# flupkede/codesearch

Hardware: AMD Instinct MI355X
Metric: chunks embedded+searched/sec over 10M×384 corpus; recall@10 vs CPU ref (higher is better)
Workload: dtype f32

## Files before the change

codesearch_amd/csrc/attention_shx_body.hpp:

```cpp
#pragma once

#include "encoder.hpp"
#include "split_f16.hpp"

#ifndef AT_STAMP
#define AT_STAMP(i)
#endif
#ifndef CS_ATTN_ARITH
#define CS_ATTN_ARITH 2
#endif
#ifndef CS_ATTN_LAZY_RESCALE
#define CS_ATTN_LAZY_RESCALE 4.0f
#endif
#ifndef CS_ATTN_PIPE_FENCE
#define CS_ATTN_PIPE_FENCE __builtin_amdgcn_sched_barrier(0)
#endif

namespace cs {

typedef __fp16 h16x2 __attribute__((ext_vector_type(2)));

constexpr float kLog2e = 1.4426950408889634f;
constexpr float kMaskedLog2 = -3.0e38f;

union Frag8 {
    f16x8 v;
    uint32_t u[4];
    uint2 d[2];
};

typedef short s16x4 __attribute__((ext_vector_type(4)));

union FragTr {
    f16x8 v;
    s16x4 q[2];
};

__device__ __forceinline__ void split_pair_rtz_ng(float a, float b, uint32_t& hi, uint32_t& lo) {
    const h16x2 h = __builtin_amdgcn_cvt_pkrtz(a, b);
    const h16x2 l = __builtin_amdgcn_cvt_pkrtz((a - (float)h[0]) * kShLoScale, (b - (float)h[1]) * kShLoScale);
    hi = __builtin_bit_cast(uint32_t, h);
    lo = __builtin_bit_cast(uint32_t, l);
}

__device__ __forceinline__ float mix_residual_lo(float e, uint32_t hpair) {
    float r;
    asm("v_fma_mix_f32 %0, %1, -1.0, %2 op_sel_hi:[1,0,0]" : "=v"(r) : "v"(hpair), "v"(e));
    return r;
}
__device__ __forceinline__ float mix_residual_hi(float e, uint32_t hpair) {
    float r;
    asm("v_fma_mix_f32 %0, %1, -1.0, %2 op_sel:[1,0,0] op_sel_hi:[1,0,0]" : "=v"(r) : "v"(hpair), "v"(e));
    return r;
}

__device__ __forceinline__ float xhalf_max_swap(float t) {
    const uint32_t u = __builtin_bit_cast(uint32_t, t);
    const auto r = __builtin_amdgcn_permlane32_swap(u, u, false, false);
    const uint32_t a = r[0], b = r[1];
    return fmaxf(__builtin_bit_cast(float, a), __builtin_bit_cast(float, b));
}

struct AttnMemPlain {
    __device__ __forceinline__ f16x8 ld16(const _Float16* p) const { return *reinterpret_cast<const f16x8*>(p); }
    __device__ __forceinline__ f16x8 stage_load(const _Float16* src, char* lds_piece) const { sh_glds16(src, lds_piece); return f16x8{}; }
    __device__ __forceinline__ void stage_store(char*, int, f16x8) const {}
    __device__ __forceinline__ void st8(_Float16* p, f16x4 v) const { *reinterpret_cast<f16x4*>(p) = v; }
};

template <int NC, class MQ, class MO, int POS = 0, int PIPE = 0>
__device__ __forceinline__ void
attention_shx_body(char* smem, const MQ& mq, const MO& mo, const _Float16* qkvs, const int32_t* __restrict__ mask,
                   _Float16* ctxs, uint32_t* __restrict__ flag, uint32_t L, uint32_t H,
                   float scale_log2e, uint32_t HB, float* __restrict__ range_out,
                   const uint32_t* __restrict__ seq_unit, const uint32_t* __restrict__ unit_len,
                   uint32_t bx, uint32_t by, uint32_t bz, uint32_t gx, uint32_t gz, const float* __restrict__ alibi_log2 = nullptr,
                   uint32_t window = 0) {
    constexpr bool ALIBI = POS == 1, WINDOW = POS == 2;
    constexpr bool IMM = PIPE >= 2;
    constexpr bool EARLY = PIPE == 3;
    const float wlimit = (float)window;
    constexpr int KT = 128;
    const uint32_t Lp = (L + 31) & ~31u;
    char* Kt = smem;
    char* Vt = Kt + (size_t)NC * KT * 128;
    float* madd = reinterpret_cast<float*>(Vt + (size_t)NC * KT * 128);
    int* last_valid_p = reinterpret_cast<int*>(madd + Lp);
    const int tid = threadIdx.x, lane = tid & 63;
    const int wave = __builtin_amdgcn_readfirstlane(tid >> 6);
    const int l31 = lane & 31, h = lane >> 5;
    const uint32_t wq = 4 / HB, hsub = (uint32_t)wave / wq, qt = (uint32_t)wave % wq;
    const uint32_t head = bx * HB + hsub, b = by, qb = bz;
    Kt += (size_t)hsub * (KT / HB) * 128;
    Vt += (size_t)hsub * (KT / HB) * 128;
    const uint32_t nh = H / (32 * NC), nch = 3 * nh * NC;
    const _Float16* base = qkvs + (size_t)b * L * nch * 64;
    bool ovf = false;

    AT_STAMP(0);
    if (tid == 0) *last_valid_p = 0;

    const int kswz = (l31 >> 1) & 7;
    int k_hi[2], k_lo[2];
#pragma unroll
    for (int s = 0; s < 2; ++s) {
        k_hi[s] = ((2 * s + h) ^ kswz) * 16;
        k_lo[s] = ((4 + 2 * s + h) ^ kswz) * 16;
    }
    const int vq = (lane & 15) >> 2, vp = lane & 3, vg = (lane >> 4) & 1;
    const int vfv = 4 * ((vq >> 1) & 1);
    const int v_hi = (4 * h + vq) * 128 + (((2 * vg + (vp >> 1)) ^ vfv) * 16) + 8 * (vp & 1);
    const int v_lo = v_hi ^ 64;

    const bool wave_live = qb * 128 + qt * 32 < L;
    const uint32_t query = qb * 128 + qt * 32 + l31;
    const uint32_t qsrc = query < L ? query : L - 1;
    float neg_slope = 0.0f;
    const float qpos = (float)query - (float)(4 * h);
    if constexpr (ALIBI) neg_slope = -alibi_log2[head];
    f16x8 qh[NC][2], ql[NC][2];
#pragma unroll
    for (int c = 0; c < NC; ++c) {
        const _Float16* qp = base + ((size_t)qsrc * nch + head * NC + c) * 64 + 8 * h;
#pragma unroll
        for (int s = 0; s < 2; ++s) {
            qh[c][s] = mq.ld16(qp + 16 * s);
            ql[c][s] = mq.ld16(qp + 32 + 16 * s);
        }
    }
#if CS_ATTN_ARITH == 2 && !defined(CS_ATTN_SCALAR_SOFTMAX)
    f16x8 qhs[NC][2];
#pragma unroll
    for (int c = 0; c < NC; ++c)
#pragma unroll
        for (int s = 0; s < 2; ++s) {
            qhs[c][s] = qh[c][s] * (_Float16)kShLoInv;
            ql[c][s] = ql[c][s] * (_Float16)kShLoInv;
        }
#endif
    sh_f32x16 ohh[NC], oxx[NC];
#pragma unroll
    for (int c = 0; c < NC; ++c)
#pragma unroll
        for (int r = 0; r < 16; ++r) { ohh[c][r] = 0.0f; oxx[c][r] = 0.0f; }
    float m = -__builtin_huge_valf(), lsum = 0.0f;

    auto stage = [&](uint32_t st) {
        const uint32_t live = Lp - st * KT < (uint32_t)KT ? Lp - st * KT : (uint32_t)KT;
        for (uint32_t i0 = qt; i0 < live / 8; i0 += 4 * wq) {
            f16x8 rk[4][NC], rv[4][NC];
#pragma unroll
            for (int u = 0; u < 4; ++u) {
                const uint32_t ii = i0 + u * wq;
                if (ii < live / 8) {
                    const uint32_t row = ii * 8 + (lane >> 3);
                    const uint32_t gk = st * KT + row;
                    const uint32_t key = gk < L ? gk : L - 1;
                    const uint32_t ck = (lane & 7) ^ ((row >> 1) & 7);
                    const uint32_t cv = (lane & 7) ^ (4 * ((row >> 1) & 1));
#pragma unroll
                    for (int c = 0; c < NC; ++c) {
                        rk[u][c] = mq.stage_load(base + ((size_t)key * nch + (nh + head) * NC + c) * 64 + ck * 8, Kt + (size_t)c * KT * 128 + ii * 1024);
                        rv[u][c] = mq.stage_load(base + ((size_t)key * nch + (2 * nh + head) * NC + c) * 64 + cv * 8, Vt + (size_t)c * KT * 128 + ii * 1024);
                    }
                }
            }
#pragma unroll
            for (int u = 0; u < 4; ++u) {
                const uint32_t ii = i0 + u * wq;
                if (ii < live / 8) {
#pragma unroll
                    for (int c = 0; c < NC; ++c) {
                        mq.stage_store(Kt + (size_t)c * KT * 128 + ii * 1024, lane, rk[u][c]);
                        mq.stage_store(Vt + (size_t)c * KT * 128 + ii * 1024, lane, rv[u][c]);
                    }
                }
            }
        }
    };
    stage(0);
    __syncthreads();
    for (uint32_t key = tid; key < Lp; key += 256) {
        const bool ok = key < L && mask[(size_t)b * L + key] != 0;
        madd[key] = ok ? 0.0f : kMaskedLog2;
        if (ok) atomicMax(last_valid_p, (int)key);
    }
    asm volatile("s_waitcnt vmcnt(0)" ::: "memory");
    __syncthreads();
    const uint32_t ntiles = (uint32_t)(*last_valid_p) / 32 + 1;

    typedef __attribute__((address_space(3))) char* lds_char_p;
    typedef __attribute__((address_space(3))) const f16x8* lds_f16x8_cp;
    typedef __attribute__((address_space(3))) const sh_f32x4* lds_f32x4_cp;
    uint32_t ka[4] = {0, 0, 0, 0}, va[2] = {0, 0}, ma0 = 0;
    if constexpr (IMM) {
        const uint32_t k0 = (uint32_t)(uintptr_t)(lds_char_p)Kt + (uint32_t)l31 * 128u, v0 = (uint32_t)(uintptr_t)(lds_char_p)Vt;
#pragma unroll
        for (int s = 0; s < 2; ++s) { ka[s] = k0 + (uint32_t)k_hi[s]; ka[2 + s] = k0 + (uint32_t)k_lo[s]; }
        va[0] = v0 + (uint32_t)v_hi;
        va[1] = v0 + (uint32_t)v_lo;
        ma0 = (uint32_t)(uintptr_t)(lds_char_p)reinterpret_cast<char*>(madd) + 16u * (uint32_t)h;
#pragma unroll
        for (int i = 0; i < 4; ++i) asm volatile("" : "+v"(ka[i]));
        asm volatile("" : "+v"(va[0]), "+v"(va[1]), "+v"(ma0));
    }

    for (uint32_t st = 0; st * 4 < ntiles; ++st) {
        if constexpr (WINDOW) {
            if (st * KT > qb * 128 + 127 + window || st * KT + (KT - 1) + window < qb * 128) continue;
        }
        if (st > 0) {
            __syncthreads();
            stage(st);
            asm volatile("s_waitcnt vmcnt(0)" ::: "memory");
            __syncthreads();
        }
        if (!wave_live) continue;
        const uint32_t kt_end = ntiles - st * 4 < 4 ? ntiles - st * 4 : 4;
        const uint32_t ma_st = ma0 + st * 512u;
        uint32_t kl_lo = 0, kl_hi = kt_end;
        if constexpr (WINDOW) {
            const int q0 = (int)(qb * 128 + qt * 32), w = (int)window, t0 = (int)(st * 4);
            const int first = q0 - 31 - w > 0 ? (q0 - 31 - w + 31) / 32 : 0, past = (q0 + 31 + w) / 32 + 1;
            kl_lo = (uint32_t)(first > t0 ? first - t0 : 0);
            kl_hi = past - t0 < (int)kt_end ? (uint32_t)(past - t0 > 0 ? past - t0 : 0) : kt_end;
        }
        auto compute_s = [&](uint32_t kl, sh_f32x16& hh, sh_f32x16& xx) __attribute__((always_inline)) {
#pragma unroll
            for (int r = 0; r < 16; ++r) { hh[r] = 0.0f; xx[r] = 0.0f; }
            if constexpr (EARLY) {
                f16x8 kf[NC][4];
#pragma unroll
                for (int c = 0; c < NC; ++c)
#pragma unroll
                    for (int i = 0; i < 4; ++i) kf[c][i] = *(lds_f16x8_cp)(uintptr_t)(ka[i] + (uint32_t)(c * KT * 128) + kl * 4096u);
                __builtin_amdgcn_sched_barrier(0);
#pragma unroll
                for (int c = 0; c < NC; ++c)
#pragma unroll
                    for (int s = 0; s < 2; ++s) {
                        hh = __builtin_amdgcn_mfma_f32_32x32x16_f16(kf[c][s], qh[c][s], hh, 0, 0, 0);
#if CS_ATTN_ARITH == 2 && !defined(CS_ATTN_SCALAR_SOFTMAX)
                        hh = __builtin_amdgcn_mfma_f32_32x32x16_f16(kf[c][s], ql[c][s], hh, 0, 0, 0);
                        hh = __builtin_amdgcn_mfma_f32_32x32x16_f16(kf[c][2 + s], qhs[c][s], hh, 0, 0, 0);
#else
                        xx = __builtin_amdgcn_mfma_f32_32x32x16_f16(kf[c][s], ql[c][s], xx, 0, 0, 0);
                        xx = __builtin_amdgcn_mfma_f32_32x32x16_f16(kf[c][2 + s], qh[c][s], xx, 0, 0, 0);
#endif
                    }
                return;
            }
#pragma unroll
            for (int c = 0; c < NC; ++c) {
                const char* kr = Kt + (size_t)c * KT * 128 + (size_t)(kl * 32 + l31) * 128;
#pragma unroll
                for (int s = 0; s < 2; ++s) {
                    f16x8 kh, kl8;
                    if constexpr (IMM) {
                        kh = *(lds_f16x8_cp)(uintptr_t)(ka[s] + (uint32_t)(c * KT * 128) + kl * 4096u);
                        kl8 = *(lds_f16x8_cp)(uintptr_t)(ka[2 + s] + (uint32_t)(c * KT * 128) + kl * 4096u);
                    } else {
                        kh = *reinterpret_cast<const f16x8*>(kr + k_hi[s]);
                        kl8 = *reinterpret_cast<const f16x8*>(kr + k_lo[s]);
                    }
                    hh = __builtin_amdgcn_mfma_f32_32x32x16_f16(kh, qh[c][s], hh, 0, 0, 0);
#if CS_ATTN_ARITH == 2 && !defined(CS_ATTN_SCALAR_SOFTMAX)
                    hh = __builtin_amdgcn_mfma_f32_32x32x16_f16(kh, ql[c][s], hh, 0, 0, 0);
                    hh = __builtin_amdgcn_mfma_f32_32x32x16_f16(kl8, qhs[c][s], hh, 0, 0, 0);
#else
                    xx = __builtin_amdgcn_mfma_f32_32x32x16_f16(kh, ql[c][s], xx, 0, 0, 0);
                    xx = __builtin_amdgcn_mfma_f32_32x32x16_f16(kl8, qh[c][s], xx, 0, 0, 0);
#endif
                }
            }
        };
        auto finish_tile = [&](uint32_t kl, sh_f32x16& hh, sh_f32x16& xx) __attribute__((always_inline)) {
            const uint32_t kt = st * 4 + kl;
#ifndef CS_ATTN_SCALAR_SOFTMAX
            sh_f32x2 p2[8];
            float tmax = -__builtin_huge_valf();
            const sh_f32x2 lo_inv2 = {kShLoInv, kShLoInv}, scale2 = {scale_log2e, scale_log2e};
#pragma unroll
            for (int g = 0; g < 4; ++g) {
                sh_f32x4 ma;
                if constexpr (IMM) ma = *(lds_f32x4_cp)(uintptr_t)(ma_st + (kl * 32u + 8u * g) * 4u);
                else ma = *reinterpret_cast<const sh_f32x4*>(madd + kt * 32 + 8 * g + 4 * h);
#pragma unroll
                for (int e2 = 0; e2 < 2; ++e2) {
                    const int r = 4 * g + 2 * e2;
                    const sh_f32x2 x2 = {xx[r], xx[r + 1]}, h2 = {hh[r], hh[r + 1]};
                    sh_f32x2 m2 = {ma[2 * e2], ma[2 * e2 + 1]};
                    if constexpr (ALIBI) {
                        const float d0 = qpos - (float)(kt * 32 + 8 * g + 2 * e2);
                        m2[0] = fmaf(neg_slope, fabsf(d0), m2[0]);
                        m2[1] = fmaf(neg_slope, fabsf(d0 - 1.0f), m2[1]);
                    }
                    if constexpr (WINDOW) {
                        const float d0 = qpos - (float)(kt * 32 + 8 * g + 2 * e2);
                        m2[0] = fabsf(d0) > wlimit ? kMaskedLog2 : m2[0];
                        m2[1] = fabsf(d0 - 1.0f) > wlimit ? kMaskedLog2 : m2[1];
                    }
#if CS_ATTN_ARITH == 2
                    (void)x2; (void)lo_inv2;
                    const sh_f32x2 s2 = __builtin_elementwise_fma(h2, scale2, m2);
#else
                    const sh_f32x2 s2 = __builtin_elementwise_fma(__builtin_elementwise_fma(x2, lo_inv2, h2), scale2, m2);
#endif
                    p2[r / 2] = s2;
                    tmax = fmaxf(tmax, fmaxf(s2[0], s2[1]));
                }
            }
            if constexpr (IMM) tmax = xhalf_max_swap(tmax);
            else tmax = fmaxf(tmax, __shfl_xor(tmax, 32, 64));
#if CS_ATTN_ARITH == 2
            if (__any(tmax > m + CS_ATTN_LAZY_RESCALE)) {
#else
            if (__any(tmax > m)) {
#endif
                const float mnew = fmaxf(m, tmax);
                const float alpha = __builtin_amdgcn_exp2f(m - mnew);
                lsum *= alpha;
#pragma unroll
                for (int c = 0; c < NC; ++c)
#pragma unroll
                    for (int r = 0; r < 16; ++r) { ohh[c][r] *= alpha; oxx[c][r] *= alpha; }
                m = mnew;
            }
            typedef __attribute__((address_space(3))) s16x4* lds_s16x4_p;
            FragTr vhe[NC][2], vle[NC][2];
            if constexpr (EARLY) {
#pragma unroll
                for (int c = 0; c < NC; ++c)
#pragma unroll
                    for (int s = 0; s < 2; ++s) {
                        const uint32_t off = (uint32_t)(c * KT * 128) + kl * 4096u + (uint32_t)(s * 16 * 128);
                        vhe[c][s].q[0] = __builtin_amdgcn_ds_read_tr16_b64_v4i16((lds_s16x4_p)(uintptr_t)(va[0] + off));
                        vhe[c][s].q[1] = __builtin_amdgcn_ds_read_tr16_b64_v4i16((lds_s16x4_p)(uintptr_t)(va[0] + off + 1024u));
                        vle[c][s].q[0] = __builtin_amdgcn_ds_read_tr16_b64_v4i16((lds_s16x4_p)(uintptr_t)(va[1] + off));
                        vle[c][s].q[1] = __builtin_amdgcn_ds_read_tr16_b64_v4i16((lds_s16x4_p)(uintptr_t)(va[1] + off + 1024u));
                    }
                __builtin_amdgcn_sched_barrier(0);
            }
#if CS_ATTN_ARITH == 2
            const sh_f32x2 m2v = {m - 11.0f, m - 11.0f};
#else
            const sh_f32x2 m2v = {m, m};
#endif
            sh_f32x2 ps2 = {0.0f, 0.0f};
            Frag8 ph[2], pl[2];
            const sh_f32x2 lo_scale2 = {kShLoScale, kShLoScale};
#pragma unroll
            for (int i = 0; i < 8; ++i) {
                const sh_f32x2 d2 = p2[i] - m2v;
                const sh_f32x2 e2 = {__builtin_amdgcn_exp2f(d2[0]), __builtin_amdgcn_exp2f(d2[1])};
                ps2 += e2;
                const h16x2 hi = __builtin_amdgcn_cvt_pkrtz(e2[0], e2[1]);
#if CS_ATTN_ARITH == 2
                (void)lo_scale2;
                const uint32_t hib = __builtin_bit_cast(uint32_t, hi);
                const h16x2 lo = __builtin_amdgcn_cvt_pkrtz(mix_residual_lo(e2[0], hib), mix_residual_hi(e2[1], hib));
#else
                const sh_f32x2 back = {(float)hi[0], (float)hi[1]};
                const sh_f32x2 r2 = (e2 - back) * lo_scale2;
                const h16x2 lo = __builtin_amdgcn_cvt_pkrtz(r2[0], r2[1]);
#endif
                ph[i >> 2].u[i & 3] = __builtin_bit_cast(uint32_t, hi);
                pl[i >> 2].u[i & 3] = __builtin_bit_cast(uint32_t, lo);
            }
            lsum += ps2[0] + ps2[1];
#else
            float tmax = -__builtin_huge_valf();
#pragma unroll
            for (int g = 0; g < 4; ++g) {
                const sh_f32x4 ma = *reinterpret_cast<const sh_f32x4*>(madd + kt * 32 + 8 * g + 4 * h);
#pragma unroll
                for (int e = 0; e < 4; ++e) {
                    const int r = 4 * g + e;
                    float me = ma[e];
                    if constexpr (ALIBI) me = fmaf(neg_slope, fabsf(qpos - (float)(kt * 32 + 8 * g + e)), me);
                    if constexpr (WINDOW) me = fabsf(qpos - (float)(kt * 32 + 8 * g + e)) > wlimit ? kMaskedLog2 : me;
                    hh[r] = fmaf(fmaf(xx[r], kShLoInv, hh[r]), scale_log2e, me);
                    tmax = fmaxf(tmax, hh[r]);
                }
            }
            tmax = fmaxf(tmax, __shfl_xor(tmax, 32, 64));
            if (__any(tmax > m)) {
                const float mnew = fmaxf(m, tmax);
                const float alpha = __builtin_amdgcn_exp2f(m - mnew);
                lsum *= alpha;
#pragma unroll
                for (int c = 0; c < NC; ++c)
#pragma unroll
                    for (int r = 0; r < 16; ++r) { ohh[c][r] *= alpha; oxx[c][r] *= alpha; }
                m = mnew;
            }
            float psum = 0.0f;
#pragma unroll
            for (int r = 0; r < 16; ++r) {
                hh[r] = __builtin_amdgcn_exp2f(hh[r] - m);
                psum += hh[r];
            }
            lsum += psum;
            Frag8 ph[2], pl[2];
#pragma unroll
            for (int s = 0; s < 2; ++s)
#pragma unroll
                for (int w2 = 0; w2 < 4; ++w2) {
#ifdef CS_ATTN_P_HI_ONLY
                    const f16x2 pr = __builtin_convertvector(sh_f32x2{hh[8 * s + 2 * w2], hh[8 * s + 2 * w2 + 1]}, f16x2);
                    ph[s].u[w2] = __builtin_bit_cast(uint32_t, pr);
                    pl[s].u[w2] = 0u;
#else
                    split_pair_rtz_ng(hh[8 * s + 2 * w2], hh[8 * s + 2 * w2 + 1], ph[s].u[w2], pl[s].u[w2]);
#endif
                }
#endif
#ifdef CS_ATTN_SCALAR_SOFTMAX
            typedef __attribute__((address_space(3))) s16x4* lds_s16x4_p;
            FragTr vhe[NC][2], vle[NC][2];
#endif
#pragma unroll
            for (int c = 0; c < NC; ++c) {
                const char* vr = Vt + (size_t)c * KT * 128 + (size_t)kl * 32 * 128;
#pragma unroll
                for (int s = 0; s < 2; ++s) {
                    FragTr vh, vl;
                    if constexpr (EARLY) {
                        vh = vhe[c][s];
                        vl = vle[c][s];
                    } else if constexpr (IMM) {
                        const uint32_t off = (uint32_t)(c * KT * 128) + kl * 4096u + (uint32_t)(s * 16 * 128);
                        vh.q[0] = __builtin_amdgcn_ds_read_tr16_b64_v4i16((lds_s16x4_p)(uintptr_t)(va[0] + off));
                        vh.q[1] = __builtin_amdgcn_ds_read_tr16_b64_v4i16((lds_s16x4_p)(uintptr_t)(va[0] + off + 1024u));
                        vl.q[0] = __builtin_amdgcn_ds_read_tr16_b64_v4i16((lds_s16x4_p)(uintptr_t)(va[1] + off));
                        vl.q[1] = __builtin_amdgcn_ds_read_tr16_b64_v4i16((lds_s16x4_p)(uintptr_t)(va[1] + off + 1024u));
                    } else {
                    vh.q[0] = __builtin_amdgcn_ds_read_tr16_b64_v4i16((lds_s16x4_p)(vr + s * 16 * 128 + v_hi));
                    vh.q[1] = __builtin_amdgcn_ds_read_tr16_b64_v4i16((lds_s16x4_p)(vr + s * 16 * 128 + 8 * 128 + v_hi));
                    vl.q[0] = __builtin_amdgcn_ds_read_tr16_b64_v4i16((lds_s16x4_p)(vr + s * 16 * 128 + v_lo));
                    vl.q[1] = __builtin_amdgcn_ds_read_tr16_b64_v4i16((lds_s16x4_p)(vr + s * 16 * 128 + 8 * 128 + v_lo));
                    }
                    ohh[c] = __builtin_amdgcn_mfma_f32_32x32x16_f16(vh.v, ph[s].v, ohh[c], 0, 0, 0);
#if CS_ATTN_ARITH == 2 && !defined(CS_ATTN_SCALAR_SOFTMAX)
                    ohh[c] = __builtin_amdgcn_mfma_f32_32x32x16_f16(vh.v, pl[s].v, ohh[c], 0, 0, 0);
#elif !defined(CS_ATTN_P_HI_ONLY)
                    oxx[c] = __builtin_amdgcn_mfma_f32_32x32x16_f16(vh.v, pl[s].v, oxx[c], 0, 0, 0);
#endif
                    oxx[c] = __builtin_amdgcn_mfma_f32_32x32x16_f16(vl.v, ph[s].v, oxx[c], 0, 0, 0);
                }
            }
        };
        if constexpr (PIPE == 0) {
            for (uint32_t kl = kl_lo; kl < kl_hi; ++kl) {
                sh_f32x16 hh, xx;
                compute_s(kl, hh, xx);
                finish_tile(kl, hh, xx);
            }
        } else if constexpr (IMM) {
#pragma unroll
            for (uint32_t kl = 0; kl < 4; ++kl) {
                if (kl >= kl_lo && kl < kl_hi) {
                    sh_f32x16 hh, xx;
                    compute_s(kl, hh, xx);
                    finish_tile(kl, hh, xx);
                }
            }
        } else {
            sh_f32x16 hhA, xxA, hhB, xxB;
            if (kl_lo < kl_hi) compute_s(kl_lo, hhA, xxA);
            for (uint32_t kl = kl_lo; kl < kl_hi; kl += 2) {
                if (kl + 1 < kl_hi) compute_s(kl + 1, hhB, xxB);
                CS_ATTN_PIPE_FENCE;
                finish_tile(kl, hhA, xxA);
                if (kl + 1 < kl_hi) {
                    if (kl + 2 < kl_hi) compute_s(kl + 2, hhA, xxA);
                    CS_ATTN_PIPE_FENCE;
                    finish_tile(kl + 1, hhB, xxB);
                }
            }
        }
    }
    lsum += __shfl_xor(lsum, 32, 64);
    const float inv = 1.0f / lsum;
    float rlo = 0.0f, rhi = 0.0f;
    if (wave_live && query < L) {
#pragma unroll
        for (int c = 0; c < NC; ++c) {
            _Float16* op = ctxs + (((size_t)b * L + query) * nh + head) * NC * 64 + c * 64 + 4 * h;
#pragma unroll
            for (int g = 0; g < 4; ++g) {
                f16x4 hi, lo;
#pragma unroll
                for (int e = 0; e < 4; ++e) {
                    _Float16 a, bb;
                    const float o = fmaf(oxx[c][4 * g + e], kShLoInv, ohh[c][4 * g + e]) * inv;
                    ovf |= sh_split(o, a, bb);
                    hi[e] = a; lo[e] = bb;
                    rlo = fminf(rlo, o);
                    rhi = fmaxf(rhi, o);
                }
                mo.st8(op + 8 * g, hi);
                mo.st8(op + 32 + 8 * g, lo);
            }
        }
    }
    AT_STAMP(2);
    if (ovf && flag) atomicOr(flag, 1u);
    if (range_out) {
        if (unit_len && query >= unit_len[seq_unit[b]]) rlo = rhi = 0.0f;
#pragma unroll
        for (int o = 32; o > 0; o >>= 1) {
            rlo = fminf(rlo, __shfl_xor(rlo, o, 64));
            rhi = fmaxf(rhi, __shfl_xor(rhi, o, 64));
        }
        if (lane == 0) {
            const size_t blk = ((size_t)by * gz + bz) * gx + bx;
            _Float16 a, bb;
            (void)sh_split(rlo, a, bb);
            range_out[(blk * 4 + wave) * 2] = fmaf((float)bb, kShLoInv, (float)a);
            (void)sh_split(rhi, a, bb);
            range_out[(blk * 4 + wave) * 2 + 1] = fmaf((float)bb, kShLoInv, (float)a);
        }
    }
}

}
```

Baseline: 4.639 billion.

## Fold softmax scale into Q and mask into MFMA accumulator init

Pre-multiplies the split-f16 query by scale_log2e and re-splits it, so the QK^T MFMA directly produces log2-scaled scores. The additive mask is loaded into the accumulator init, which removes the per-element fma in the softmax path. Tile max uses an inline-asm v_max3 chain, and the last-valid-key search uses a wave ballot instead of per-lane atomics. Risks include precision changes from re-splitting the scaled Q and hand-written s_nop hazard padding for reading MFMA results.

```diff
diff --git a/codesearch_amd/csrc/attention_shx_body.hpp b/codesearch_amd/csrc/attention_shx_body.hpp
--- a/codesearch_amd/csrc/attention_shx_body.hpp
+++ b/codesearch_amd/csrc/attention_shx_body.hpp
@@ -60,6 +60,31 @@
     const uint32_t a = r[0], b = r[1];
     return fmaxf(__builtin_bit_cast(float, a), __builtin_bit_cast(float, b));
 }
+
+#define CS_ATTN_MAX3_CHAIN                                                                                                     \
+    "v_max3_f32 %0, %2, %3, %4\n\tv_max3_f32 %0, %0, %5, %6\n\tv_max3_f32 %0, %0, %7, %8\n\tv_max3_f32 %0, %0, %9, %10\n\t"      \
+    "v_max3_f32 %0, %0, %11, %12\n\tv_max3_f32 %0, %0, %13, %14\n\tv_max3_f32 %0, %0, %15, %16\n\tv_max3_f32 %0, %0, %17, %17\n\t"
+#define CS_ATTN_MAX_XHALF "v_mov_b32 %1, %0\n\ts_nop 1\n\tv_permlane32_swap_b32 %0, %1\n\tv_max_f32 %0, %0, %1"
+#define CS_ATTN_MAX_OPERANDS(t, u, a)                                                                                          \
+    "=&v"(t), "=&v"(u)                                                                                                         \
+        : "v"(a[0]), "v"(a[1]), "v"(a[2]), "v"(a[3]), "v"(a[4]), "v"(a[5]), "v"(a[6]), "v"(a[7]), "v"(a[8]), "v"(a[9]), "v"(a[10]), \
+          "v"(a[11]), "v"(a[12]), "v"(a[13]), "v"(a[14]), "v"(a[15])
+template <bool FROM_MFMA, bool XHALF>
+__device__ __forceinline__ float tile_max16(const sh_f32x16& a) {
+    float t, u;
+    if constexpr (FROM_MFMA && XHALF) asm("s_nop 11\n\t" CS_ATTN_MAX3_CHAIN CS_ATTN_MAX_XHALF : CS_ATTN_MAX_OPERANDS(t, u, a));
+    else if constexpr (FROM_MFMA) asm("s_nop 11\n\t" CS_ATTN_MAX3_CHAIN "v_mov_b32 %1, %0" : CS_ATTN_MAX_OPERANDS(t, u, a));
+    else if constexpr (XHALF) asm(CS_ATTN_MAX3_CHAIN CS_ATTN_MAX_XHALF : CS_ATTN_MAX_OPERANDS(t, u, a));
+    else asm(CS_ATTN_MAX3_CHAIN "v_mov_b32 %1, %0" : CS_ATTN_MAX_OPERANDS(t, u, a));
+    if constexpr (!XHALF) {
+        const float o = __shfl_xor(u, 32, 64);
+        asm("v_max_f32 %0, %1, %2" : "=v"(t) : "v"(t), "v"(o));
+    }
+    return t;
+}
+#undef CS_ATTN_MAX3_CHAIN
+#undef CS_ATTN_MAX_XHALF
+#undef CS_ATTN_MAX_OPERANDS
 
 struct AttnMemPlain {
     __device__ __forceinline__ f16x8 ld16(const _Float16* p) const { return *reinterpret_cast<const f16x8*>(p); }
@@ -134,6 +159,12 @@
     for (int c = 0; c < NC; ++c)
 #pragma unroll
         for (int s = 0; s < 2; ++s) {
+#pragma unroll
+            for (int j = 0; j < 8; ++j) {
+                _Float16 a, bb;
+                (void)sh_split(fmaf((float)ql[c][s][j], kShLoInv, (float)qh[c][s][j]) * scale_log2e, a, bb);
+                qh[c][s][j] = a; ql[c][s][j] = bb;
+            }
             qhs[c][s] = qh[c][s] * (_Float16)kShLoInv;
             ql[c][s] = ql[c][s] * (_Float16)kShLoInv;
         }
@@ -180,11 +211,14 @@
     };
     stage(0);
     __syncthreads();
+    int wave_last = 0;
     for (uint32_t key = tid; key < Lp; key += 256) {
         const bool ok = key < L && mask[(size_t)b * L + key] != 0;
         madd[key] = ok ? 0.0f : kMaskedLog2;
-        if (ok) atomicMax(last_valid_p, (int)key);
-    }
+        const unsigned long long okb = __ballot(ok);
+        if (okb) wave_last = (int)(key - (uint32_t)lane) + 63 - __builtin_clzll(okb);
+    }
+    if (lane == 0 && wave_last > 0) atomicMax(last_valid_p, wave_last);
     asm volatile("s_waitcnt vmcnt(0)" ::: "memory");
     __syncthreads();
     const uint32_t ntiles = (uint32_t)(*last_valid_p) / 32 + 1;
@@ -226,8 +260,19 @@
             kl_hi = past - t0 < (int)kt_end ? (uint32_t)(past - t0 > 0 ? past - t0 : 0) : kt_end;
         }
         auto compute_s = [&](uint32_t kl, sh_f32x16& hh, sh_f32x16& xx) __attribute__((always_inline)) {
+#if CS_ATTN_ARITH == 2 && !defined(CS_ATTN_SCALAR_SOFTMAX)
+#pragma unroll
+            for (int g = 0; g < 4; ++g) {
+                sh_f32x4 ma;
+                if constexpr (IMM) ma = *(lds_f32x4_cp)(uintptr_t)(ma_st + (kl * 32u + 8u * g) * 4u);
+                else ma = *reinterpret_cast<const sh_f32x4*>(madd + (st * 4 + kl) * 32 + 8 * g + 4 * h);
+#pragma unroll
+                for (int e = 0; e < 4; ++e) { hh[4 * g + e] = ma[e]; xx[4 * g + e] = 0.0f; }
+            }
+#else
 #pragma unroll
             for (int r = 0; r < 16; ++r) { hh[r] = 0.0f; xx[r] = 0.0f; }
+#endif
             if constexpr (EARLY) {
                 f16x8 kf[NC][4];
 #pragma unroll
@@ -278,6 +323,22 @@
             const uint32_t kt = st * 4 + kl;
 #ifndef CS_ATTN_SCALAR_SOFTMAX
             sh_f32x2 p2[8];
+#if CS_ATTN_ARITH == 2
+            (void)xx;
+            if constexpr (ALIBI || WINDOW) {
+#pragma unroll
+                for (int g = 0; g < 4; ++g)
+#pragma unroll
+                    for (int e = 0; e < 4; ++e) {
+                        const float d = fabsf(qpos - (float)(kt * 32 + 8 * g + e));
+                        if constexpr (ALIBI) hh[4 * g + e] = fmaf(neg_slope, d, hh[4 * g + e]);
+                        else hh[4 * g + e] = d > wlimit ? kMaskedLog2 : hh[4 * g + e];
+                    }
+            }
+            const float tmax = tile_max16<POS == 0, IMM>(hh);
+#pragma unroll
+            for (int i = 0; i < 8; ++i) p2[i] = sh_f32x2{hh[2 * i], hh[2 * i + 1]};
+#else
             float tmax = -__builtin_huge_valf();
             const sh_f32x2 lo_inv2 = {kShLoInv, kShLoInv}, scale2 = {scale_log2e, scale_log2e};
 #pragma unroll
@@ -300,18 +361,14 @@
                         m2[0] = fabsf(d0) > wlimit ? kMaskedLog2 : m2[0];
                         m2[1] = fabsf(d0 - 1.0f) > wlimit ? kMaskedLog2 : m2[1];
                     }
-#if CS_ATTN_ARITH == 2
-                    (void)x2; (void)lo_inv2;
-                    const sh_f32x2 s2 = __builtin_elementwise_fma(h2, scale2, m2);
-#else
                     const sh_f32x2 s2 = __builtin_elementwise_fma(__builtin_elementwise_fma(x2, lo_inv2, h2), scale2, m2);
-#endif
                     p2[r / 2] = s2;
                     tmax = fmaxf(tmax, fmaxf(s2[0], s2[1]));
                 }
             }
             if constexpr (IMM) tmax = xhalf_max_swap(tmax);
             else tmax = fmaxf(tmax, __shfl_xor(tmax, 32, 64));
+#endif
 #if CS_ATTN_ARITH == 2
             if (__any(tmax > m + CS_ATTN_LAZY_RESCALE)) {
 #else
@@ -351,9 +408,18 @@
             const sh_f32x2 lo_scale2 = {kShLoScale, kShLoScale};
 #pragma unroll
             for (int i = 0; i < 8; ++i) {
+#ifdef CS_ATTN_SCALAR_ADDS
+                float d0 = p2[i][0] - m2v[0], d1 = p2[i][1] - m2v[1];
+                asm volatile("" : "+v"(d0), "+v"(d1));
+                const sh_f32x2 e2 = {__builtin_amdgcn_exp2f(d0), __builtin_amdgcn_exp2f(d1)};
+                ps2[0] += e2[0];
+                ps2[1] += e2[1];
+                asm volatile("" : "+v"(ps2[0]), "+v"(ps2[1]));
+#else
                 const sh_f32x2 d2 = p2[i] - m2v;
                 const sh_f32x2 e2 = {__builtin_amdgcn_exp2f(d2[0]), __builtin_amdgcn_exp2f(d2[1])};
                 ps2 += e2;
+#endif
                 const h16x2 hi = __builtin_amdgcn_cvt_pkrtz(e2[0], e2[1]);
 #if CS_ATTN_ARITH == 2
                 (void)lo_scale2;
```

Measured after the change: 4.638 billion. About the same (-0.0%).
